# kekley/octree_pathtracing

Measured on AMD Instinct MI355X. Metric: Mrays/sec at 1920×1080×256spp; achieved HBM GB/s vs roofline at 1/2/4/8 GPUs, higher is better.
Workload: dtype f32

## Files before the change

octree_pathtracing_amd/csrc/octpt_api.cpp:

```cpp
#include <hip/hip_runtime.h>

#include <algorithm>
#include <atomic>
#include <chrono>
#include <cmath>
#include <cstdlib>
#include <thread>
#include <cstdio>
#include <cstring>
#include <new>
#include <string>
#include <memory>
#include <vector>

#include "../../include/octpt.h"
#include "octpt_internal.h"
#include "octpt_mask.h"
#include "octpt_reproject.h"

using namespace octpt;

namespace {

constexpr uint32_t kCounterRing = 256;
constexpr uint64_t kMaxChunkPaths = 1ull << 31;
constexpr uint64_t kDefaultChunkPaths = 1ull << 29;
#ifndef OCTPT_LOOKAHEAD
#define OCTPT_LOOKAHEAD 3
#endif
constexpr uint32_t kLookahead = OCTPT_LOOKAHEAD;
constexpr uint32_t kDefaultPool = 512u << 20;
constexpr uint32_t kMaxPool = 1u << 30;
constexpr uint32_t kMinPool = 1u << 20;
constexpr uint32_t kDefaultRefill = 0;
constexpr uint32_t kDefaultDrainRays = 4096;
#ifndef OCTPT_SAMPLE_GROUP_DEFAULT
#define OCTPT_SAMPLE_GROUP_DEFAULT 4
#endif
constexpr uint32_t kDefaultSampleGroup = OCTPT_SAMPLE_GROUP_DEFAULT;
constexpr uint64_t kGroupMinItems = 1ull << 27;

uint32_t group_shift_of(uint32_t most, uint32_t chunk_spp) {
    uint32_t g = 6u;
    while (g && ((1u << g) > most || chunk_spp % (1u << g) != 0u)) g -= 2u;
    return g;
}

uint32_t env_u32(const char *name, uint32_t dflt) {
    const char *v = std::getenv(name);
    if (!v || !*v) return dflt;
    const long x = std::strtol(v, nullptr, 10);
    return x > 0 ? (uint32_t)x : dflt;
}

struct EventPair {
    hipEvent_t start, stop;
};

template <class T>
struct DevBuf {
    T *p = nullptr;
    size_t n = 0;
};

}

struct octpt_ctx {
    int device = 0;
    int num_cu = 0;
    hipStream_t stream = nullptr;
    std::string err;
    bool has_scene = false;
    DevScene S{};
    std::vector<void *> scene_allocs;
    bool has_camera = false;
    octpt_camera cam{};
    DevCamera C{};
    uint32_t *d_counters = nullptr;
    std::vector<uint2> h_subs;
    uint2 *d_subs = nullptr;
    size_t subs_cap = 0;
    float *d_beam = nullptr;
    size_t beam_cap = 0;
    uint32_t launch_seq = 0;
    unsigned long long *d_stats = nullptr;
    uint8_t *d_lut_byte = nullptr;
    float *d_lut_float = nullptr;
    std::vector<EventPair> pending;
    double kernel_ms = 0.0;
    uint64_t launches = 0;
    bool ktiming = false;
    std::vector<std::pair<int, EventPair>> kpending;
    std::vector<EventPair> ev_pool;
    double kern_ms[2] = {0.0, 0.0};
    uint64_t kern_n[2] = {0, 0};
    float build_ms = 0.0f;
    BuildScratch build_scratch;
    int blocks_per_cu_cache[kMaxDepth + 1] = {0};
    int extend_bpc_cache[kMaxDepth + 1][4] = {};
    int shade_bpc_cache[2][2][3] = {};
    bool lean_scene = false;
    bool no_lean = false;
    bool sample_group_set = false;
    uint32_t sample_group = kDefaultSampleGroup;
    WaveBuffers wb{};
    size_t pool = 0, color_cap = 0, nee_pool = 0;
    void *nee_alloc = nullptr;
    std::vector<void *> wave_allocs;
    void *color_alloc = nullptr;
    size_t wave_bytes = 0, mem_limit = 0;
    std::vector<std::pair<void *, size_t>> wave_sizes;
    uint64_t wave_allocs_n = 0;
    bool oom_warned = false;
    uint32_t *h_count = nullptr;
    uint32_t *d_count = nullptr;
    hipEvent_t count_ev[kLookahead + 1] = {};
    uint32_t pool_cap = kDefaultPool, refill = kDefaultRefill;
    bool beam = true;
    uint32_t drain_rays = kDefaultDrainRays;
    bool drain_models = false;
    uint64_t chunk_cap = kDefaultChunkPaths;
    octpt_frame *inflight = nullptr;
    std::vector<octpt_ctx *> sub;
    float4 *m_acc = nullptr;
    uint32_t *m_seg = nullptr;
    size_t m_acc_cap = 0, m_seg_cap = 0;
    float4 *dn_frame[2] = {nullptr, nullptr};
    size_t dn_cap[2] = {0, 0};
    std::vector<uint32_t> h_order;
    uint32_t order_w = 0, order_h = 0;
    uint32_t *d_order = nullptr, *d_order_pos = nullptr;
    uint64_t scene_gen = 0, camera_gen = 0, order_gen = 0;
    struct BeamKey {
        uint64_t scene = 0, camera = 0, order = 0;
        uint64_t list = 0;
        uint32_t w = 0, h = 0, shard_index = 0, shard_count = 0;
        bool valid = false;
        bool operator==(const BeamKey &o) const {
            return valid && o.valid && scene == o.scene && camera == o.camera && order == o.order && list == o.list &&
                   w == o.w && h == o.h && shard_index == o.shard_index && shard_count == o.shard_count;
        }
    } beam_key;
    uint32_t *d_tiles = nullptr;
    size_t tiles_cap = 0;
    uint64_t list_gen = 0;
    uint32_t *d_tile_spp = nullptr;
    float *d_tile_err = nullptr;
    size_t tile_spp_cap = 0, tile_err_cap = 0;
    float sample_clamp = 0.0f;
    float *d_tile_spread = nullptr;
    size_t tile_spread_cap = 0;
    float4 *fin_normal = nullptr, *fin_albedo = nullptr;
    float *fin_depth = nullptr, *fin_var = nullptr;
    size_t fin_normal_cap = 0, fin_albedo_cap = 0, fin_depth_cap = 0, fin_var_cap = 0;
    hipEvent_t beam_ev = nullptr;
    hipStream_t beam_stream = nullptr;
    bool beam_shared = false;
};

struct octpt_frame {
    octpt_ctx *ctx = nullptr;
    octpt_render_params params{};
    std::thread worker;
    std::atomic<bool> finished{false};
    std::atomic<bool> cancel_requested{false};
    octpt_status status = OCTPT_OK;
    float *user_accum = nullptr;
    uint8_t *user_rgba = nullptr;
    size_t n_pixels = 0;
    float4 *d_accum = nullptr;
    uchar4 *d_rgba = nullptr;
    float *h_accum = nullptr;
    uint8_t *h_rgba = nullptr;
    bool delivered = false;
};

namespace {

octpt_status fail(octpt_ctx *ctx, octpt_status st, const std::string &msg) {
    if (ctx) ctx->err = msg;
    return st;
}

octpt_status hip_fail(octpt_ctx *ctx, hipError_t e, const char *what) {
    return fail(ctx, e == hipErrorOutOfMemory ? OCTPT_ERR_OOM : OCTPT_ERR_DEVICE,
                std::string(what) + ": " + hipGetErrorString(e));
}

#define HIP_TRY(ctx, expr)                                 \
    do {                                                   \
// ... 3155 lines not shown
```

octree_pathtracing_amd/csrc/octpt_kernels.hip:

```cpp
#include "octpt_internal.h"
#include "octpt_rcp.h"
#include "octpt_reproject.h"

#ifndef OCTPT_RCP_FAST
#define OCTPT_RCP_FAST 1
#endif

namespace octpt {
namespace {

#define RAY_EPSILON 0.00000005f
#define RAY_OFFSET 0.000001f
#define OCTREE_MAX_STEPS 1000u
#define OCTREE_MAX_SCALE 23u
#define OCTREE_EPSILON 1.1920929e-7f
#define MAX_DST_WORLD 1024.0f
#define PI_F 3.14159265358979323846f
#define CELL_TOL 0.001f
#define SUN_MAX_CHANCE 0.9f
#define MAT_FLAG_REFRACTIVE 0x4u
#define MAT_FLAG_SUBSURFACE 0x2u
#define MAX_PATH_SEGMENTS 64u
constexpr uint32_t kBeamIterBits = 10u;
constexpr uint32_t kBeamIterMask = (1u << kBeamIterBits) - 1u;
static_assert(OCTREE_MAX_STEPS <= kBeamIterMask + 1u, "the skipped-iteration bound fits its bits");

struct v3 {
    float x, y, z;
};
__device__ __forceinline__ v3 V(float x, float y, float z) { return v3{x, y, z}; }
__device__ __forceinline__ v3 vadd(v3 a, v3 b) { return V(a.x + b.x, a.y + b.y, a.z + b.z); }
__device__ __forceinline__ v3 vsub(v3 a, v3 b) { return V(a.x - b.x, a.y - b.y, a.z - b.z); }
__device__ __forceinline__ v3 vmul(v3 a, v3 b) { return V(a.x * b.x, a.y * b.y, a.z * b.z); }
__device__ __forceinline__ v3 vscale(v3 a, float s) { return V(a.x * s, a.y * s, a.z * s); }
__device__ __forceinline__ float vdot(v3 a, v3 b) { return (a.x * b.x + a.y * b.y) + a.z * b.z; }
__device__ __forceinline__ v3 vcross(v3 a, v3 b) {
    return V(a.y * b.z - b.y * a.z, a.z * b.x - b.z * a.x, a.x * b.y - b.x * a.y);
}
__device__ __forceinline__ v3 vnorm(v3 a) {
    float r = 1.0f / sqrtf(vdot(a, a));
    return vscale(a, r);
}
__device__ __forceinline__ float fmn(float a, float b) { return a < b ? a : b; }
__device__ __forceinline__ float fmx(float a, float b) { return a > b ? a : b; }
__device__ __forceinline__ float vmin3(v3 a) { return fmn(fmn(a.x, a.y), a.z); }
__device__ __forceinline__ float vmax3(v3 a) { return fmx(fmx(a.x, a.y), a.z); }
__device__ __forceinline__ float tmn(float a, float b) { return __builtin_fminf(a, b); }
__device__ __forceinline__ float tmx(float a, float b) { return __builtin_fmaxf(a, b); }
__device__ __forceinline__ float tmin3(v3 a) { return tmn(tmn(a.x, a.y), a.z); }
__device__ __forceinline__ float tmn_nc(float a, float b) {
    float r;
    asm("v_min_f32 %0, %1, %2" : "=v"(r) : "v"(a), "v"(b));
    return r;
}
__device__ __forceinline__ float tmax3(v3 a) { return tmx(tmx(a.x, a.y), a.z); }
__device__ __forceinline__ float signum_(float f) { return (__float_as_uint(f) >> 31) ? -1.0f : 1.0f; }

__device__ __forceinline__ void dm_sincos(float x, float &s, float &c) {
    const float kf = floorf(x * 0.636619772367581343f + 0.5f);
    const int k = (int)kf;
    const float r = ((x - kf * 1.5703125f) - kf * 4.837512969970703125e-4f) - kf * 7.54978995489188216e-8f;
    const float z = r * r;
    const float sp = r + r * z * (-1.6666654611e-1f + z * (8.3321608736e-3f + z * -1.9515295891e-4f));
    const float cp = (1.0f - 0.5f * z) +
                     z * z * (4.166664568298827e-2f + z * (-1.388731625493765e-3f + z * 2.443315711809948e-5f));
    switch (k & 3) {
    case 0: s = sp; c = cp; break;
    case 1: s = cp; c = -sp; break;
    case 2: s = -sp; c = -cp; break;
    default: s = -cp; c = sp; break;
    }
}
__device__ __forceinline__ float dm_cos(float x) { float s, c; dm_sincos(x, s, c); return c; }

__device__ inline float dm_asin(float x) {
    const float a = fabsf(x);
    float z, xx;
    bool flag = false;
    if (a > 0.5f) {
        z = 0.5f * (1.0f - a);
        xx = sqrtf(z);
        flag = true;
    } else {
        xx = a;
        z = a * a;
    }
    float r;
    if (a < 1.0e-4f && !flag) {
        r = xx;
    } else {
        r = ((((4.2163199048e-2f * z + 2.4181311049e-2f) * z + 4.5470025998e-2f) * z + 7.4953002686e-2f) * z +
             1.6666752422e-1f) * z * xx + xx;
    }
    if (flag) {
        r = r + r;
        r = 1.5707963267948966f - r;
    }
    return x < 0.0f ? -r : r;
}
__device__ inline float dm_acos(float x) {
    if (x < -0.5f) return PI_F - 2.0f * dm_asin(sqrtf(0.5f * (1.0f + x)));
    if (x > 0.5f) return 2.0f * dm_asin(sqrtf(0.5f * (1.0f - x)));
    return 1.5707963267948966f - dm_asin(x);
}
__device__ inline float dm_atan_core(float x) {
    float sgn = 1.0f, y;
    if (x < 0.0f) { sgn = -1.0f; x = -x; }
    if (x > 2.414213562373095f) {
        y = 1.5707963267948966f;
        x = -1.0f / x;
    } else if (x > 0.4142135623730950f) {
        y = 0.7853981633974483f;
        x = (x - 1.0f) / (x + 1.0f);
    } else {
        y = 0.0f;
    }
    const float z = x * x;
    y = y + ((((8.05374449538e-2f * z - 1.38776856032e-1f) * z + 1.99777106478e-1f) * z - 3.33329491539e-1f) * z * x + x);
    return sgn < 0.0f ? -y : y;
}
__device__ inline float dm_atan2(float y, float x) {
    int code = 0;
    if (x < 0.0f) code = 2;
    if (y < 0.0f) code |= 1;
    if (x == 0.0f) {
        if (code & 1) return -1.5707963267948966f;
        if (y == 0.0f) return 0.0f;
        return 1.5707963267948966f;
    }
    if (y == 0.0f) return (code & 2) ? PI_F : 0.0f;
    float w = 0.0f;
    if (code == 2) w = PI_F;
    else if (code == 3) w = -PI_F;
    return w + dm_atan_core(y / x);
}
__device__ __forceinline__ float dm_hypot(float x, float y) { return sqrtf(x * x + y * y); }

__device__ __forceinline__ uint32_t lowbias32(uint32_t x) {
    x ^= x >> 16; x *= 0x7feb352du; x ^= x >> 15; x *= 0x846ca68bu; x ^= x >> 16;
    return x;
}
__device__ __forceinline__ uint32_t path_state(uint32_t seed, uint32_t pixel, uint32_t sample) {
    uint32_t h = lowbias32(seed ^ 0xA511E9B3u);
    h = lowbias32(h ^ pixel);
    return lowbias32(h ^ (sample * 0x9E3779B9u));
}
__device__ __forceinline__ float rng_next(uint32_t &st) {
    const uint32_t s = st * 747796405u + 2891336453u;
    st = s;
    uint32_t w = ((s >> ((s >> 28u) + 4u)) ^ s) * 277803737u;
    w = (w >> 22u) ^ w;
    return (float)(w >> 8) * (1.0f / 16777216.0f);
}

__device__ __forceinline__ uint32_t branch_state(uint32_t state, uint32_t b) {
// ... 1355 lines not shown
    Counters cnt = {0u, 0u, 0u, 0u, 0u, 0u, 0u};
    const uint32_t item = blockIdx.x * kBlock + threadIdx.x;
    uint32_t x = 0u, y = 0u;
    if (item < R.total_items) item_pixel(R, item, x, y);
    if (item < R.total_items && x < R.W && y < R.H) {
        const uint32_t pix = y * R.W + x;
        PathState ps;
        const float xn = ((float)(2u * x + 1u) - (float)R.W) / R.dim;
        const float yn = ((float)(2u * (R.H - y) - 1u) - (float)R.H) / R.dim;
        const v3 nd = vadd(vadd(vscale(V(C.dir[0], C.dir[1], C.dir[2]), C.d_factor),
                                vscale(V(C.right[0], C.right[1], C.right[2]), xn)),
                           vscale(V(C.up[0], C.up[1], C.up[2]), yn));
        ps.o = V(C.eye[0], C.eye[1], C.eye[2]);
        ps.d = vnorm(nd);
        ps.n = V(0.0f, 0.0f, 0.0f);
        ps.col[0] = ps.col[1] = ps.col[2] = ps.col[3] = 0.0f;
        ps.T = V(1.0f, 1.0f, 1.0f);
        ps.L = V(0.0f, 0.0f, 0.0f);
        ps.cur = ps.prev = ps.depth = 0u;
        ps.rng = 0u;
        ps.last_prim = kPrimNone;
        ps.path_segs = 0u;
        ps.specular = true;
        cnt.paths++;
        uint32_t pix_segs = 0u;
        while (begin_segment(ps)) {
            cnt.segs++;
            pix_segs++;
            const TraceRay tr = trace_ray_of(S, ps);
            Esvo E;
            esvo_begin(S, tr, E, stk);
            uint32_t prim = kPrimNone;
            PrimHit h;
            int rs;
            do {
                rs = esvo_step<kPrims>(S, tr, E, stk, cnt, prim, h);
            } while (rs == kStepContinue);
            cnt.steps += E.iter;
            if (rs != kStepHit) break;
            commit_hit(S, ps, prim, h, cnt);
            if (ps.cur != 0u && ps.col[3] > 0.0f) break;
            ps.o = vadd(ps.o, vscale(ps.d, RAY_OFFSET));
        }
        float out[3];
        if (ps.cur == 0u) {
            sky_color(S.sun, ps, out);
        } else {
            const float shading = fmaxf(0.3f, vdot(ps.n, V(S.sun.sw[0], S.sun.sw[1], S.sun.sw[2])));
            for (int i = 0; i < 3; ++i) out[i] = ps.col[i] * (S.sun.emit[i] * shading);
        }
        const uint32_t ai = R.compact ? item : pix;
        float4 fb = accum[ai];
        fb.x = out[0];
        fb.y = out[1];
        fb.z = out[2];
        accum[ai] = fb;
        if (segcount) segcount[ai] += pix_segs;
    }
    cnt.ib = 0u;
    flush_counters(cnt, stats);
}

constexpr uint32_t kRayBeamBit = 0x40000000u;
constexpr uint32_t kHitCapped = 1u;
__device__ __forceinline__ void store_ray(const WaveBuffers &B, uint32_t q, uint32_t pos, uint32_t slot,
                                          const PathState &ps) {
    const bool beam = ps.beam > 0.0f && ps.path_segs == 1u;
    B.ray0[q][pos] = make_float4(ps.o.x, ps.o.y, ps.o.z, beam ? ps.beam : __uint_as_float(ps.last_prim));
    B.ray1[q][pos] = make_float4(ps.d.x, ps.d.y, ps.d.z,
                                 __uint_as_float(slot | (vdot(ps.d, ps.n) < 0.0f ? 0x80000000u : 0u) |
                                                 (beam ? kRayBeamBit : 0u)));
}
__device__ __forceinline__ void store_cam_ray(const WaveBuffers &B, uint32_t pos, const PathState &ps) {
    B.ray1[0][pos] = make_float4(ps.d.x, ps.d.y, ps.d.z, ps.beam > 0.0f ? ps.beam : 0.0f);
}
__device__ __forceinline__ void cam_ray(float4 eye, uint32_t slot, float4 &r0, float4 &r1) {
    const float b = r1.w;
    r0 = make_float4(eye.x, eye.y, eye.z, b > 0.0f ? b : eye.w);
    r1.w = __uint_as_float(slot | (b > 0.0f ? kRayBeamBit : 0u));
}
__device__ __forceinline__ uint32_t ray_last_prim(float4 r0, float4 r1) {
    return (__float_as_uint(r1.w) & kRayBeamBit) ? kPrimNone : __float_as_uint(r0.w);
}
__device__ __forceinline__ float ray_beam(float4 r0, float4 r1) {
    return (__float_as_uint(r1.w) & kRayBeamBit) ? r0.w : 0.0f;
}

__device__ __forceinline__ void pack_path(const PathState &ps, uint32_t item, float4 &a, float4 &b, uint2 &c) {
    a = make_float4(ps.T.x, ps.T.y, ps.T.z, ps.L.x);
    b = make_float4(ps.L.y, ps.L.z, __uint_as_float(ps.rng), __uint_as_float(item));
    c = make_uint2(ps.cur, ps.depth | (ps.specular ? 1u << 8 : 0u) | (ps.shadow ? 1u << 9 : 0u) | (ps.branch << 10) |
                               (ps.path_segs << 16) | (ps.seg_base << 23));
}
__device__ __forceinline__ void store_path(const WaveBuffers &B, uint32_t slot, const PathState &ps, uint32_t item) {
    float4 a, b;
    uint2 c;
    pack_path(ps, item, a, b, c);
    B.pa[slot] = a;
    B.pb[slot] = b;
    B.pc[slot] = c;
}

__device__ __forceinline__ void store_lean_at(const WaveBuffers &B, uint32_t q, uint32_t pos, const PathState &ps) {
    float4 a, b;
    uint2 c;
    pack_path(ps, 0u, a, b, c);
    (q ? B.pb : B.pa)[pos] = make_float4(a.x, a.y, a.z, b.z);
    B.pc[(size_t)q * kSegs * B.seg_cap + pos] = c;
}

__device__ __forceinline__ void store_nee(const WaveBuffers &B, uint32_t slot, const PathState &ps) {
    B.pd[slot] = make_float4(ps.co.x, ps.co.y, ps.co.z, __uint_as_float(ps.clast));
    B.pd[B.pool + slot] = make_float4(ps.cd.x, ps.cd.y, ps.cd.z, __uint_as_float(ps.ccur));
    B.pd[2u * B.pool + slot] = make_float4(ps.cn.x, ps.cn.y, ps.cn.z, ps.mult);
}
__device__ __forceinline__ void store_att(const WaveBuffers &B, uint32_t slot, const PathState &ps) {
    B.pd[3u * B.pool + slot] = make_float4(ps.att[0], ps.att[1], ps.att[2], ps.att[3]);
}
__device__ __forceinline__ void load_nee(const WaveBuffers &B, uint32_t slot, PathState &ps) {
    const float4 a = B.pd[slot], b = B.pd[B.pool + slot], c = B.pd[2u * B.pool + slot], d = B.pd[3u * B.pool + slot];
    ps.co = V(a.x, a.y, a.z);
    ps.clast = __float_as_uint(a.w);
    ps.cd = V(b.x, b.y, b.z);
    ps.ccur = __float_as_uint(b.w);
    ps.cn = V(c.x, c.y, c.z);
    ps.mult = c.w;
    ps.att[0] = d.x; ps.att[1] = d.y; ps.att[2] = d.z; ps.att[3] = d.w;
}

__device__ __forceinline__ void unpack_path(float4 a, float4 b, uint2 c, float4 r0, float4 r1, PathState &ps,
                                            uint32_t &item) {
    ps.o = V(r0.x, r0.y, r0.z);
    ps.last_prim = ray_last_prim(r0, r1);
    ps.d = V(r1.x, r1.y, r1.z);
    ps.beam = 0.0f;
    ps.T = V(a.x, a.y, a.z);
    ps.L = V(a.w, b.x, b.y);
    ps.rng = __float_as_uint(b.z);
    item = __float_as_uint(b.w);
    ps.cur = c.x;
    ps.prev = c.x;
    ps.depth = c.y & 255u;
    ps.specular = (c.y >> 8) & 1u;
    ps.shadow = (c.y >> 9) & 1u;
    ps.branch = (c.y >> 10) & 63u;
    ps.path_segs = (c.y >> 16) & 127u;
    ps.seg_base = c.y >> 23;
}
__device__ __forceinline__ void load_path(const WaveBuffers &B, uint32_t slot, float4 r0, float4 r1, PathState &ps,
                                          uint32_t &item) {
    unpack_path(B.pa[slot], B.pb[slot], B.pc[slot], r0, r1, ps, item);
}

__device__ __forceinline__ uint32_t group_swap(uint32_t v, uint32_t pos, uint32_t low) {
    const uint32_t mid = (v >> pos) & 7u;
    return (v & ~(7u << pos)) | ((((mid & ((1u << low) - 1u)) << (3u - low)) | (mid >> low)) << pos);
}
template <bool kFastDiv = true>
__device__ __forceinline__ void item_split(const DevRender &R, uint32_t item, uint32_t &s_local, uint32_t &px_item) {
    const uint32_t g = R.group_shift;
    const uint32_t n = item >> g;
    const uint32_t sg = kFastDiv ? udiv_c(n, R.div_items) : n / R.total_items;
    const uint32_t pq = n - sg * R.total_items;
    s_local = (sg << g) | (item & ((1u << g) - 1u));
    px_item = g ? group_swap(pq, 3u - (g >> 1), 3u - (g >> 1)) : pq;
}
__device__ __forceinline__ size_t item_of(const DevRender &R, uint32_t s_local, uint32_t pq) {
    const uint32_t g = R.group_shift;
    return (((size_t)(s_local >> g) * R.total_items + pq) << g) + (s_local & ((1u << g) - 1u));
}

template <bool kFastDiv = true>
__device__ __forceinline__ bool item_path(const DevCamera &C, const DevRender &R, uint32_t item, PathState &ps,
                                          uint32_t &x, uint32_t &y) {
    uint32_t s_local, px_item;
    item_split<kFastDiv>(R, item, s_local, px_item);
    item_pixel<kFastDiv>(R, px_item, x, y);
    if (x >= R.W || y >= R.H) return false;
    uint32_t sample = R.spp_start + s_local, branch = 0u;
    if (R.subs) {
        const uint2 sb = R.subs[s_local];
        sample = sb.x;
        branch = sb.y >> 16;
    }
    new_path(C, R, x, y, sample, ps);
    ps.branch = branch;
    begin_segment(ps);
    return true;
}

template <bool kSeed = false>
__device__ inline bool seed_item(const DevCamera &C, const DevRender &R, const WaveBuffers &B, uint32_t slot,
                                 uint32_t item, PathState &ps, Counters &cnt) {
    uint32_t x, y;
    if (!item_path(C, R, item, ps, x, y)) {
        B.color[item] = make_float4(0.0f, 0.0f, 0.0f, 0.0f);
        return false;
    }
    cnt.paths++;
    if (R.beam)
        ps.beam = R.beam[(y / kBeamTile) * R.beam_tx + x / kBeamTile];
    if (kSeed) {
        if (!B.lean) B.item0[slot] = item;
    } else {
        store_path(B, slot, ps, item);
    }
    return true;
}

static_assert(kSegs == 64, "segment scans give one wave lane per segment");

__device__ __forceinline__ uint32_t relaxed_load(const uint32_t *p) {
    return __hip_atomic_load(p, __ATOMIC_RELAXED, __HIP_MEMORY_SCOPE_AGENT);
}
__device__ __forceinline__ uint32_t shard_lo(uint32_t k, uint32_t n) {
    return (uint32_t)(((uint64_t)k * n) / kSegs);
}
__device__ __forceinline__ uint32_t first_from(uint64_t m, uint32_t from) {
    const uint64_t r = from ? ((m >> from) | (m << (64u - from))) : m;
    return (from + (uint32_t)__ffsll((unsigned long long)r) - 1u) & 63u;
}

struct ItemCursor {
    uint32_t k;
    bool left;
};

template <bool kSeed = false>
__device__ inline bool regen(const DevCamera &C, const DevRender &R, const WaveBuffers &B, uint32_t slot, bool want,
                             uint32_t chunk_items, ItemCursor &cur, PathState &ps, Counters &cnt) {
    bool need = want, ok = false;
    while (cur.left && __ballot(need) != 0ull) {
        const uint32_t lo = shard_lo(cur.k, chunk_items), n = shard_lo(cur.k + 1u, chunk_items) - lo;
        const uint32_t t = wave_ticket(B.ctrl + ctr_item(cur.k), need);
        bool dry = false;
        if (need) {
            if (t >= n) dry = true;
            else if (seed_item<kSeed>(C, R, B, slot, lo + t, ps, cnt)) { ok = true; need = false; }
        }
        if (__ballot(dry) != 0ull) {
            const uint32_t j = threadIdx.x & 63u;
            const bool has = relaxed_load(B.ctrl + ctr_item(j)) < shard_lo(j + 1u, chunk_items) - shard_lo(j, chunk_items);
            const uint64_t m = __ballot(has);
            cur.left = m != 0ull;
            if (cur.left) cur.k = first_from(m, cur.k);
        }
    }
    return ok;
}

__global__ __launch_bounds__(kBlock) void wf_seed_kernel(DevCamera C, DevRender R, WaveBuffers B, uint32_t n_seed,
                                                         uint32_t chunk_items, unsigned long long *__restrict__ stats) {
    const uint32_t i = blockIdx.x * kBlock + threadIdx.x;
    const uint32_t seg = (i >> 6) % kSegs;
    Counters cnt = {0u, 0u, 0u, 0u, 0u, 0u, 0u};
    PathState ps;
    bool ok = false;
    uint32_t slot = i;
    if (n_seed == chunk_items) {
        if (blockIdx.x == 0u && threadIdx.x < kSegs)
            B.ctrl[ctr_item(threadIdx.x)] = shard_lo(threadIdx.x + 1u, chunk_items) - shard_lo(threadIdx.x, chunk_items);
        const uint32_t lo = shard_lo(seg, chunk_items), hi = shard_lo(seg + 1u, chunk_items);
        const uint32_t item = lo + (i >> 6) / kSegs * 64u + (i & 63u);
        slot = item;
        if (item < hi) ok = seed_item<true>(C, R, B, slot, item, ps, cnt);
        if (((R.W | R.H) & (kTile - 1u)) == 0u) {
            if (blockIdx.x == 0u && threadIdx.x < kSegs)
                B.ctrl[ctr_count(0u, threadIdx.x)] = shard_lo(threadIdx.x + 1u, chunk_items) - shard_lo(threadIdx.x, chunk_items);
            if (ok) store_cam_ray(B, seg * B.seg_cap + (item - lo), ps);
            if (blockIdx.x == 0u && threadIdx.x == 0u) B.ray0[0][0] = B.eye;
            if (blockIdx.x == 0u && threadIdx.x == 0u) atomicAdd(&stats[kStatPaths], (unsigned long long)chunk_items);
            return;
        }
    } else {
        ItemCursor cur = {seg, true};
        ok = regen<true>(C, R, B, i, i < n_seed, chunk_items, cur, ps, cnt);
    }
    const uint32_t t = wave_ticket(B.ctrl + ctr_count(0u, seg), ok);
    if (ok) store_ray(B, 0u, seg * B.seg_cap + t, slot, ps);
    flush_counters(cnt, stats);
}

#ifndef OCTPT_SPH_WAVES
#define OCTPT_SPH_WAVES 8
#endif
#ifndef OCTPT_BOX_WAVES
#define OCTPT_BOX_WAVES 7
#endif
#ifndef OCTPT_MDL_WAVES
#define OCTPT_MDL_WAVES 6
#endif
#ifndef OCTPT_BLK_WAVES
#define OCTPT_BLK_WAVES 6
#endif
#define OCTPT_EXTEND_WAVES_OF(k)                                                                              \
    ((k) == kPrimsSpheres ? OCTPT_SPH_WAVES                                                                   \
                          : (k) == kPrimsBoxes ? OCTPT_BOX_WAVES : (k) == kPrimsBlocks ? OCTPT_BLK_WAVES : OCTPT_MDL_WAVES)
#ifndef OCTPT_CLAIM
#define OCTPT_CLAIM 64
#endif
constexpr uint32_t kClaim = OCTPT_CLAIM;
static_assert(kSegs % 8u == 0u, "eight XCDs share the segments evenly");
#ifndef OCTPT_THR_LONG
#define OCTPT_THR_LONG 16
#endif
#ifndef OCTPT_THR_SHORT
#define OCTPT_THR_SHORT 32
#endif
#ifndef OCTPT_SHORT_STEPS
#define OCTPT_SHORT_STEPS 48
// ... 237 lines not shown
        if (valid) {
            float4 r1 = B.ray1[q][i];
            if (first == 2u) {
                float4 r0c;
                cam_ray(B.eye, shard_lo(seg, chunk_items) + base + lane, r0c, r1);
            }
            const float4 r0 = first ? B.eye : B.ray0[q][i];
            append = shade_lane<kNee, kMode == 2, kSP>(S, C, R, B, first != 0u, r0, r1, B.hit + i,
                                                  S.has_blocks ? B.hit4 + i : nullptr, ps, slot, item, cnt, q, i);
            finished = !append;
        }
        if constexpr (kMode == 1) {
            if (regen(C, R, B, slot, finished, chunk_items, cur, ps, cnt)) append = true;
        }
        const uint32_t t = wave_ticket(B.ctrl + ctr_count(q ^ 1u, seg), append);
        if (append) {
            store_ray(B, q ^ 1u, seg0 + t, slot, ps);
            if constexpr (kMode == 2) store_lean_at(B, q ^ 1u, seg0 + t, ps);
        }
    }
    cnt.ib = 0u;
    flush_counters(cnt, stats);
}

template <int kPrims, bool kNee>
__global__ __launch_bounds__(kBlock) void wf_drain_kernel(DevScene S, DevRender R, WaveBuffers B, uint32_t q,
                                                          unsigned long long *__restrict__ stats) {
    extern __shared__ uint2 lds_stack[];
    const Stack stk = stack_of(lds_stack, S.depth);
    Counters cnt = {0u, 0u, 0u, 0u, 0u, 0u, 0u};
    const uint32_t wid = (blockIdx.x * kBlock + threadIdx.x) >> 6, nw = (gridDim.x * kBlock) >> 6;
    const uint32_t jlim = (threadIdx.x & 63u) == 0u ? 0xFFFFFFFFu : 0u;
    for (uint32_t k = 0; k < kSegs; ++k) {
        const uint32_t n = min(B.ctrl[ctr_count(q, k)], jlim);
        for (uint32_t j = wid; j < n; j += nw) {
            const uint32_t p = k * B.seg_cap + j;
            float4 r0 = B.ray0[q][p], r1 = B.ray1[q][p];
            for (;;) {
                const TraceRay tr = make_trace_ray(S, V(r0.x, r0.y, r0.z), V(r1.x, r1.y, r1.z), ray_last_prim(r0, r1),
                                                   (__float_as_uint(r1.w) >> 31) != 0u);
                Esvo E;
                esvo_begin(S, tr, E, stk, ray_beam(r0, r1));
                cnt.steps -= E.iter;
                bool beam_ray = (__float_as_uint(r1.w) & kRayBeamBit) != 0u;
                uint32_t prim = kPrimNone;
                PrimHit h;
                int rs;
                for (;;) {
                    do {
                        HIT_POISON(prim, h);
                        rs = esvo_step<kPrims, true>(S, tr, E, stk, cnt, prim, h);
                        SLOT_CHECK(E, stats, kStatDrainRow);
                    } while (rs == kStepContinue);
                    HIT_CHECK(kPrims, rs, prim, h, stats, kStatDrainRow);
                    cnt.steps += E.iter;
                    if (!((rs == kStepMiss) & esvo_capped(E.iter) & beam_ray)) break;
                    cnt.redo++;
                    beam_ray = false;
                    esvo_root(S, E);
                    esvo_first_child(E);
                }
                cnt.segs++;
                uint2 hr;
                if constexpr (kPrims == kPrimsBlocks)
                    hr = rs == kStepHit ? make_uint2(prim, __float_as_uint(h.t)) : make_uint2(kPrimNone, 0u);
                else
                    hr = rs == kStepHit ? hit_record(prim, h) : make_uint2(kPrimNone, 0u);
                const uint4 h4 = make_uint4(hr.x, hr.y, __float_as_uint(h.u), __float_as_uint(h.v));
                PathState ps;
                uint32_t slot, item;
                const bool lean = !kNee && B.lean;
                const bool cont = lean ? shade_lane<kNee, true>(S, DevCamera{}, R, B, false, r0, r1, &hr, &h4, ps, slot, item,
                                                                cnt, q, p)
                                       : shade_lane<kNee, false>(S, DevCamera{}, R, B, false, r0, r1, &hr, &h4, ps, slot, item, cnt);
                if (!cont) break;
                if (lean) store_lean_at(B, q, p, ps);
                r0 = make_float4(ps.o.x, ps.o.y, ps.o.z, __uint_as_float(ps.last_prim));
                r1 = make_float4(ps.d.x, ps.d.y, ps.d.z,
                                 __uint_as_float(slot | (vdot(ps.d, ps.n) < 0.0f ? 0x80000000u : 0u)));
            }
        }
    }
    flush_counters(cnt, stats, kStatDrainRow);
}

__device__ __forceinline__ float luminance(float r, float g, float b);

__device__ __forceinline__ void running_moments(float2 &m, v3 c, uint32_t spp, uint32_t bc) {
    const float s_inv = 1.0f / (float)(bc + spp);
    const float fs = (float)spp, w = (float)bc;
    const float l = luminance(c.x, c.y, c.z);
    m.x = (m.x * fs + l * w) * s_inv;
    m.y = (m.y * fs + (l * l) * w) * s_inv;
}

__device__ __forceinline__ v3 clamp_sample(v3 c, float clamp) {
    const float l = luminance(c.x, c.y, c.z);
    if (l > clamp) {
        const float k = clamp / l;
        c = V(c.x * k, c.y * k, c.z * k);
    }
    return c;
}

template <bool kMoments, bool kClamp>
__device__ __forceinline__ void resolve_pixel(const DevRender &R, const WaveBuffers &B, uint32_t chunk_spp,
                                              float4 *__restrict__ accum, uint32_t *__restrict__ segcount,
                                              float2 *__restrict__ moments, float clamp) {
    const uint32_t px_item = blockIdx.x * kBlock + threadIdx.x;
    if (px_item >= R.total_items) return;
    uint32_t x, y;
    item_pixel(R, px_item, x, y);
    if (x >= R.W || y >= R.H) return;
    const uint32_t acc_idx = R.compact ? px_item : y * R.W + x;
    float4 fb = accum[acc_idx];
    float2 mo = make_float2(0.0f, 0.0f);
    if constexpr (kMoments) mo = moments[acc_idx];
    uint32_t segs = 0u;
    v3 L0 = V(0.0f, 0.0f, 0.0f), sum = L0;
    bool split = false;
    const uint32_t gh = R.group_shift >> 1;
    const uint32_t pq = gh ? group_swap(px_item, 3u - gh, gh) : px_item;
    for (uint32_t s = 0; s < chunk_spp; ++s) {
        const float4 c = B.color[item_of(R, s, pq)];
        const uint32_t w = __float_as_uint(c.w);
        segs += w & 0x7FFFFFFFu;
        if (!R.subs) {
            v3 cs = V(c.x, c.y, c.z);
            if constexpr (kClamp) cs = clamp_sample(cs, clamp);
            running_mean(fb, cs, R.spp_start + s, 1u);
            if constexpr (kMoments) running_moments(mo, cs, R.spp_start + s, 1u);
            continue;
        }
        const uint2 sb = R.subs[s];
        const uint32_t b = sb.y >> 16, bc = sb.y & 0xFFFFu;
        if (b == 0u) {
            L0 = V(c.x, c.y, c.z);
            sum = vadd(V(0.0f, 0.0f, 0.0f), L0);
            split = (w >> 31) != 0u;
        } else {
            sum = vadd(sum, V(c.x, c.y, c.z));
        }
        if (b + 1u == bc) {
            const float inv = 1.0f / (float)bc;
            v3 folded = split ? vscale(sum, inv) : L0;
            if constexpr (kClamp) folded = clamp_sample(folded, clamp);
            running_mean(fb, folded, sb.x, bc);
            if constexpr (kMoments) running_moments(mo, folded, sb.x, bc);
        }
    }
    accum[acc_idx] = fb;
    if constexpr (kMoments) moments[acc_idx] = mo;
    if (segcount) segcount[acc_idx] += segs;
}

__global__ __launch_bounds__(kBlock) void wf_resolve_kernel(DevRender R, WaveBuffers B, uint32_t chunk_spp,
                                                            float4 *__restrict__ accum, uint32_t *__restrict__ segcount) {
    resolve_pixel<false, false>(R, B, chunk_spp, accum, segcount, nullptr, 0.0f);
}

__global__ __launch_bounds__(kBlock) void wf_resolve_moments_kernel(DevRender R, WaveBuffers B, uint32_t chunk_spp,
                                                                    float4 *__restrict__ accum,
                                                                    uint32_t *__restrict__ segcount,
                                                                    float2 *__restrict__ moments) {
    resolve_pixel<true, false>(R, B, chunk_spp, accum, segcount, moments, 0.0f);
}

__global__ __launch_bounds__(kBlock) void wf_resolve_clamp_kernel(DevRender R, WaveBuffers B, uint32_t chunk_spp,
                                                                  float4 *__restrict__ accum,
                                                                  uint32_t *__restrict__ segcount, float clamp) {
    resolve_pixel<false, true>(R, B, chunk_spp, accum, segcount, nullptr, clamp);
}

__global__ __launch_bounds__(kBlock) void wf_resolve_moments_clamp_kernel(DevRender R, WaveBuffers B, uint32_t chunk_spp,
                                                                          float4 *__restrict__ accum,
                                                                          uint32_t *__restrict__ segcount,
                                                                          float2 *__restrict__ moments, float clamp) {
    resolve_pixel<true, true>(R, B, chunk_spp, accum, segcount, moments, clamp);
}

template <int kPrims>
__global__ __launch_bounds__(kBlock) void intersect_kernel(DevScene S, const float *__restrict__ rays,
                                                           const uint32_t *__restrict__ last_prim,
                                                           const float *__restrict__ last_normal, uint32_t n,
                                                           float *__restrict__ out_t, uint32_t *__restrict__ out_prim,
                                                           float *__restrict__ out_normal, uint32_t *__restrict__ out_steps) {
    extern __shared__ uint2 lds_stack[];
    const Stack stk = stack_of(lds_stack, S.depth);
    const uint32_t i = blockIdx.x * kBlock + threadIdx.x;
    if (i >= n) return;
    PathState ps;
    ps.o = V(rays[6 * i], rays[6 * i + 1], rays[6 * i + 2]);
    ps.d = V(rays[6 * i + 3], rays[6 * i + 4], rays[6 * i + 5]);
    ps.n = last_normal ? V(last_normal[3 * i], last_normal[3 * i + 1], last_normal[3 * i + 2]) : V(0.0f, 0.0f, 0.0f);
    ps.cur = ps.prev = ps.depth = 0u;
    ps.last_prim = last_prim ? last_prim[i] : kPrimNone;
    ps.specular = true;
    const TraceRay tr = trace_ray_of(S, ps);
    Esvo E;
    Counters cnt = {0u, 0u, 0u, 0u, 0u, 0u, 0u};
    esvo_begin(S, tr, E, stk);
    uint32_t prim = kPrimNone;
    PrimHit h;
    int rs;
    do {
        rs = esvo_step<kPrims>(S, tr, E, stk, cnt, prim, h);
    } while (rs == kStepContinue);
    if (rs == kStepHit) {
        commit_hit(S, ps, prim, h, cnt);
        out_t[i] = h.t;
        out_prim[i] = kPrims != kPrimsBlocks ? prim : ((prim & kPrimCuboidBit) ? kQuadKey | (prim & kPrimIndexMask)
                                                                                 : prim & kPrimIndexMask);
        if (out_normal) {
            out_normal[3 * i] = ps.n.x;
            out_normal[3 * i + 1] = ps.n.y;
            out_normal[3 * i + 2] = ps.n.z;
        }
    } else {
        out_t[i] = __int_as_float(0x7f800000);
        out_prim[i] = kPrimNone;
        if (out_normal) out_normal[3 * i] = out_normal[3 * i + 1] = out_normal[3 * i + 2] = 0.0f;
    }
    if (out_steps) out_steps[i] = E.iter;
}

constexpr int kBeamLevels = 24;
static_assert(kTile % kBeamTile == 0, "beam tiles nest in the 8x8 render tiles");
constexpr uint32_t kBeamSub = (kTile / kBeamTile) * (kTile / kBeamTile);
__host__ __device__ constexpr uint32_t beam_levels(uint32_t depth) {
    return depth < 1u ? 1u : depth < (uint32_t)kBeamLevels ? depth : (uint32_t)kBeamLevels;
}
#ifndef OCTPT_BEAM_VISITS
#define OCTPT_BEAM_VISITS (1u << 13)
#endif
constexpr uint32_t kBeamVisits = OCTPT_BEAM_VISITS;
#ifndef OCTPT_BEAM_LOD
#define OCTPT_BEAM_LOD 0.0f
#endif
constexpr float kBeamLod = OCTPT_BEAM_LOD;
constexpr float kBeamEsvoSlack = 0x1p-21f;

__device__ __forceinline__ float beam_pack(float t, uint32_t nodes) {
    const uint32_t bound = 4u * nodes;
    const uint32_t b = __float_as_uint(t);
    if (bound >= OCTREE_MAX_STEPS || b < 2u * (kBeamIterMask + 1u)) return 0.0f;
    return __uint_as_float(((b - (kBeamIterMask + 1u)) & ~kBeamIterMask) | bound);
}

constexpr uint32_t kBeamLanes = 8u;
__global__ __launch_bounds__(64) void beam_kernel(DevScene S, DevCamera C, DevRender R, uint32_t n_tiles,
                                                  float *__restrict__ beam) {
    const uint32_t lane = threadIdx.x & (kBeamLanes - 1u), grp = threadIdx.x / kBeamLanes;
    const uint32_t i = blockIdx.x * (64u / kBeamLanes) + grp;
    if (i >= n_tiles) return;
    const uint32_t rt = dealt_tile(R.tile_order, R.shard_index + (i / kBeamSub) * R.shard_count), sub = i % kBeamSub;
    const uint32_t rty = udiv_c(rt, R.div_tiles_x);
    const uint32_t x0 = (rt - rty * R.tiles_x) * kTile + (sub % (kTile / kBeamTile)) * kBeamTile,
                   y0 = rty * kTile + (sub / (kTile / kBeamTile)) * kBeamTile;
    if (x0 >= R.W || y0 >= R.H) return;
    const uint32_t tile = (y0 / kBeamTile) * R.beam_tx + x0 / kBeamTile;
    const uint32_t x1 = min(x0 + kBeamTile, R.W), y1 = min(y0 + kBeamTile, R.H);
    float s0 = ((float)(2u * x0) - (float)R.W) / R.dim, s1 = ((float)(2u * x1) - (float)R.W) / R.dim;
    float t0 = ((float)(2u * (R.H - y1)) - (float)R.H) / R.dim, t1 = ((float)(2u * (R.H - y0)) - (float)R.H) / R.dim;
    const float ps = 0.02f * (s1 - s0) + 1e-6f, pt = 0.02f * (t1 - t0) + 1e-6f;
    s0 -= ps; s1 += ps; t0 -= pt; t1 += pt;
    const v3 F = vscale(V(C.dir[0], C.dir[1], C.dir[2]), C.d_factor);
    const v3 Rt = V(C.right[0], C.right[1], C.right[2]), Up = V(C.up[0], C.up[1], C.up[2]);
    const v3 Ek[4] = {vadd(vadd(F, vscale(Rt, s0)), vscale(Up, t0)), vadd(vadd(F, vscale(Rt, s1)), vscale(Up, t0)),
                      vadd(vadd(F, vscale(Rt, s1)), vscale(Up, t1)), vadd(vadd(F, vscale(Rt, s0)), vscale(Up, t1))};
    const v3 Ec = vadd(vadd(F, vscale(Rt, 0.5f * (s0 + s1))), vscale(Up, 0.5f * (t0 + t1)));
    v3 pn[4];
    for (int k = 0; k < 4; ++k) {
        v3 n = vcross(Ek[k], Ek[(k + 1) & 3]);
        if (vdot(n, Ec) < 0.0f) n = vscale(n, -1.0f);
        pn[k] = n;
    }
    const v3 e = vadd(vscale(V(C.eye[0], C.eye[1], C.eye[2]), S.octree_scale), V(1.0f, 1.0f, 1.0f));
    const float slack = kBeamEsvoSlack * (4.0f + fmaxf(fmaxf(fabsf(e.x), fabsf(e.y)), fabsf(e.z)));
    auto box = [&](v3 lo, float h) -> float {
        const v3 a = vsub(lo, e), b = vsub(vadd(lo, V(h, h, h)), e);
        const float ext = fmaxf(fmaxf(fmaxf(fabsf(a.x), fabsf(b.x)), fmaxf(fabsf(a.y), fabsf(b.y))),
                                fmaxf(fabsf(a.z), fabsf(b.z)));
        for (int k = 0; k < 4; ++k) {
            const v3 n = pn[k];
            const float mx = (fmaxf(n.x * a.x, n.x * b.x) + fmaxf(n.y * a.y, n.y * b.y)) + fmaxf(n.z * a.z, n.z * b.z);
            const float tol = (1e-5f * ext + slack) * ((fabsf(n.x) + fabsf(n.y)) + fabsf(n.z));
            if (mx < -tol) return -1.0f;
        }
        const float dx = a.x > 0.0f ? a.x : (b.x < 0.0f ? -b.x : 0.0f);
        const float dy = a.y > 0.0f ? a.y : (b.y < 0.0f ? -b.y : 0.0f);
        const float dz = a.z > 0.0f ? a.z : (b.z < 0.0f ? -b.z : 0.0f);
        return sqrtf((dx * dx + dy * dy) + dz * dz);
    };
    const float lod = kBeamLod * fmaxf(s1 - s0, t1 - t0) / sqrtf(vdot(F, F));
    float best = __builtin_inff();
    extern __shared__ uint32_t beam_lds[];
    const uint32_t t = threadIdx.x, L = beam_levels(S.depth);
    constexpr uint32_t G = 64u / kBeamLanes;
    float *const st_d = reinterpret_cast<float *>(beam_lds);
    uint32_t *const st_base = beam_lds + L * 64u, *const st_mask = st_base + L * G;
    float *const st_lx = reinterpret_cast<float *>(st_mask + L * G), *const st_ly = st_lx + L * G, *const st_lz = st_ly + L * G;
    auto grp_min = [](uint32_t k) {
        k = min(k, (uint32_t)__builtin_amdgcn_update_dpp((int)k, (int)k, 0xB1, 0xF, 0xF, false));
        k = min(k, (uint32_t)__builtin_amdgcn_update_dpp((int)k, (int)k, 0x4E, 0xF, 0xF, false));
        k = min(k, (uint32_t)__builtin_amdgcn_update_dpp((int)k, (int)k, 0x141, 0xF, 0xF, false));
        return k;
// ... 625 lines not shown

hipError_t launch_denoise_prep(uint32_t W, uint32_t H, const float4 *color, const float4 *albedo, const float *depth,
                               float4 *sig, hipStream_t stream) {
    const uint32_t n = W * H;
    hipLaunchKernelGGL(denoise_prep_kernel, dim3((n + 255u) / 256u), dim3(256), 0, stream, n, color, albedo, depth, sig);
    return hipGetLastError();
}

hipError_t launch_atrous(const DevDenoise &D, uint32_t iter, bool last, const float4 *src, float4 *dst,
                         hipStream_t stream) {
    const dim3 grid((D.W + kDnX - 1u) / kDnX, (D.H + kDnY - 1u) / kDnY);
    hipLaunchKernelGGL(last ? atrous_kernel<true> : atrous_kernel<false>, grid, dim3(256), 0, stream, D, iter, src, dst);
    return hipGetLastError();
}

hipError_t launch_temporal(const DevTemporal &T, bool moments, hipStream_t stream) {
    const dim3 grid((T.W + kDnX - 1u) / kDnX, (T.H + kDnY - 1u) / kDnY);
    hipLaunchKernelGGL(moments ? temporal_kernel<true> : temporal_kernel<false>, grid, dim3(256), 0, stream, T);
    return hipGetLastError();
}

hipError_t launch_variance(const DevVariance &V, hipStream_t stream) {
    const dim3 grid((V.W + kDnX - 1u) / kDnX, (V.H + kDnY - 1u) / kDnY);
    hipLaunchKernelGGL(variance_kernel, grid, dim3(256), 0, stream, V);
    return hipGetLastError();
}

hipError_t launch_denoise_var_prep(uint32_t W, uint32_t H, const float4 *color, const float *variance,
                                   const float4 *albedo, const float *depth, float4 *sig, hipStream_t stream) {
    const uint32_t n = W * H;
    hipLaunchKernelGGL(denoise_var_prep_kernel, dim3((n + 255u) / 256u), dim3(256), 0, stream, n, color, variance, albedo,
                       depth, sig);
    return hipGetLastError();
}

hipError_t launch_atrous_var(const DevDenoiseVar &D, uint32_t iter, bool last, const float4 *src, float4 *dst,
                             hipStream_t stream) {
    const dim3 grid((D.W + kDnX - 1u) / kDnX, (D.H + kDnY - 1u) / kDnY);
    hipLaunchKernelGGL(last ? atrous_var_kernel<true> : atrous_var_kernel<false>, grid, dim3(256), 0, stream, D, iter, src,
                       dst);
    return hipGetLastError();
}

hipError_t launch_render(const DevScene &S0, const DevCamera &C, const DevRender &R, float4 *accum, uint32_t *segcount,
                         uint32_t *counter, unsigned long long *stats, int grid, hipStream_t stream) {
    const DevScene &S = S0;
    auto kern = S.sun.sun_sampling ? (S.has_blocks ? render_kernel<true, kPrimsBlocks> : render_kernel<true, kPrimsModels>)
                                   : (S.has_blocks ? render_kernel<false, kPrimsBlocks> : render_kernel<false, kPrimsModels>);
    hipLaunchKernelGGL(kern, dim3(grid), dim3(kBlock), render_lds_bytes(S.depth), stream, S, C, R, accum, segcount,
                       counter, stats);
    return hipGetLastError();
}

hipError_t launch_wf_seed(const DevCamera &C, const DevRender &R, const WaveBuffers &B, uint32_t n_seed,
                          uint32_t chunk_items, unsigned long long *stats, hipStream_t stream) {
    const uint64_t threads = n_seed == chunk_items
                                 ? (uint64_t)kSegs * ((((uint64_t)chunk_items + kSegs - 1u) / kSegs + 63u) / 64u) * 64u
                                 : (uint64_t)n_seed;
    hipLaunchKernelGGL(wf_seed_kernel, dim3((uint32_t)((threads + kBlock - 1u) / kBlock)), dim3(kBlock), 0, stream, C, R, B, n_seed,
                       chunk_items, stats);
    return hipGetLastError();
}

hipError_t launch_wf_extend(const DevScene &S, const WaveBuffers &B, uint32_t q, bool cam, uint32_t refill, int grid,
                            unsigned long long *stats, hipStream_t stream) {
    uint32_t rf = refill | (cam ? 0x80000000u : 0u);
    void *args[] = {const_cast<DevScene *>(&S), const_cast<WaveBuffers *>(&B), &q, &rf, &stats};
    const hipError_t e = hipLaunchKernel(extend_instance(S), dim3(grid), dim3(kBlock), args, render_lds_bytes(S.depth),
                                         stream);
    if (e != hipSuccess) return e;
    return hipGetLastError();
}

template <bool kLds, int kSP>
static const void *lean_shade_of(bool first) {
    return !first ? reinterpret_cast<const void *>(wf_shade_kernel<false, kLds, 2, true, kSP>)
                  : reinterpret_cast<const void *>(wf_shade_kernel<false, kLds, 2, false, kSP>);
}
template <bool kNee, bool kLds>
static const void *shade_instance_of(int mode, bool first, int prims) {
    if (!kNee && mode == 2) {
        if (prims == kShadeSphColour) return lean_shade_of<kLds, kShadeSphColour>(first);
        if (prims == kPrimsSpheres) return lean_shade_of<kLds, kPrimsSpheres>(first);
        if (prims == kPrimsBoxes) return lean_shade_of<kLds, kPrimsBoxes>(first);
        if (prims == kPrimsBlocks) return lean_shade_of<kLds, kPrimsBlocks>(first);
        return lean_shade_of<kLds, kPrimsModels>(first);
    }
    return mode == 1 ? reinterpret_cast<const void *>(wf_shade_kernel<kNee, kLds, 1>)
                     : reinterpret_cast<const void *>(wf_shade_kernel<kNee, kLds, 0>);
}
bool shade_lds_tables(const DevScene &S) { return S.n_mats <= kShadeLdsMats && S.n_texs <= kShadeLdsMats; }
static const void *shade_instance(const DevScene &S, int mode, bool first = false) {
    const bool lds = shade_lds_tables(S);
    const int prims = S.has_blocks    ? kPrimsBlocks
                      : S.has_models  ? kPrimsModels
                      : S.has_cuboids ? kPrimsBoxes
                      : S.has_images  ? kPrimsSpheres
                                      : kShadeSphColour;
    return S.sun.sun_sampling
               ? (lds ? shade_instance_of<true, true>(mode, first, prims) : shade_instance_of<true, false>(mode, first, prims))
               : (lds ? shade_instance_of<false, true>(mode, first, prims) : shade_instance_of<false, false>(mode, first, prims));
}

int shade_blocks_per_cu(const DevScene &S, int mode) {
    int blocks = 0;
    if (hipOccupancyMaxActiveBlocksPerMultiprocessor(&blocks, shade_instance(S, mode), kBlock, 0) != hipSuccess)
        return 4;
    return blocks > 0 ? blocks : 1;
}

hipError_t launch_wf_shade(const DevScene &S, const DevCamera &C, const DevRender &R, const WaveBuffers &B, uint32_t q,
                           uint32_t chunk_items, uint32_t first, bool regen, int grid, unsigned long long *stats,
                           hipStream_t stream) {
    uint32_t first_u = first;
    void *args[] = {const_cast<DevScene *>(&S), const_cast<DevCamera *>(&C), const_cast<DevRender *>(&R),
                    const_cast<WaveBuffers *>(&B), &q, &chunk_items, &first_u, &stats};
    const hipError_t e = hipLaunchKernel(shade_instance(S, shade_mode(regen, B.lean != 0u), first != 0u), dim3(grid),
                                         dim3(kBlock), args, 0, stream);
    if (e != hipSuccess) return e;
    return hipGetLastError();
}

hipError_t launch_wf_drain(const DevScene &S, const DevRender &R, const WaveBuffers &B, uint32_t q, int grid,
                           unsigned long long *stats, hipStream_t stream) {
    const bool nee = S.sun.sun_sampling != 0;
    const void *fn = S.has_blocks ? (nee ? reinterpret_cast<const void *>(wf_drain_kernel<kPrimsBlocks, true>)
                                         : reinterpret_cast<const void *>(wf_drain_kernel<kPrimsBlocks, false>))
                     : S.has_models ? (nee ? reinterpret_cast<const void *>(wf_drain_kernel<kPrimsModels, true>)
                                         : reinterpret_cast<const void *>(wf_drain_kernel<kPrimsModels, false>))
                     : S.has_cuboids ? (nee ? reinterpret_cast<const void *>(wf_drain_kernel<kPrimsBoxes, true>)
                                            : reinterpret_cast<const void *>(wf_drain_kernel<kPrimsBoxes, false>))
                                     : (nee ? reinterpret_cast<const void *>(wf_drain_kernel<kPrimsSpheres, true>)
                                            : reinterpret_cast<const void *>(wf_drain_kernel<kPrimsSpheres, false>));
    void *args[] = {const_cast<DevScene *>(&S), const_cast<DevRender *>(&R), const_cast<WaveBuffers *>(&B), &q, &stats};
    const hipError_t e = hipLaunchKernel(fn, dim3(grid), dim3(kBlock), args, render_lds_bytes(S.depth), stream);
    if (e != hipSuccess) return e;
    return hipGetLastError();
}

__global__ __launch_bounds__(2 * kSegs) void wf_snapshot_kernel(const uint32_t *__restrict__ ctrl, uint32_t q,
                                                                uint32_t *__restrict__ host_out) {
    const uint32_t t = threadIdx.x;
    host_out[t] = ctrl[t < kSegs ? ctr_count(q, t) : ctr_item(t - kSegs)];
}

hipError_t launch_wf_snapshot(const WaveBuffers &B, uint32_t q, uint32_t *host_out, hipStream_t stream) {
    hipLaunchKernelGGL(wf_snapshot_kernel, dim3(1), dim3(2 * kSegs), 0, stream, B.ctrl, q, host_out);
    return hipGetLastError();
}

hipError_t launch_wf_resolve(const DevRender &R, const WaveBuffers &B, uint32_t chunk_spp, float4 *accum,
                             uint32_t *segcount, float2 *moments, float clamp, hipStream_t stream) {
    const dim3 grid((R.total_items + kBlock - 1u) / kBlock);
    if (clamp != 0.0f) {
        if (moments)
            hipLaunchKernelGGL(wf_resolve_moments_clamp_kernel, grid, dim3(kBlock), 0, stream, R, B, chunk_spp, accum,
                               segcount, moments, clamp);
        else
            hipLaunchKernelGGL(wf_resolve_clamp_kernel, grid, dim3(kBlock), 0, stream, R, B, chunk_spp, accum, segcount,
                               clamp);
    } else if (moments)
        hipLaunchKernelGGL(wf_resolve_moments_kernel, grid, dim3(kBlock), 0, stream, R, B, chunk_spp, accum, segcount,
                           moments);
    else
        hipLaunchKernelGGL(wf_resolve_kernel, grid, dim3(kBlock), 0, stream, R, B, chunk_spp, accum, segcount);
    return hipGetLastError();
}

hipError_t launch_adaptive_init(uint32_t n, float4 *accum, float2 *moments, hipStream_t stream) {
    hipLaunchKernelGGL(adaptive_init_kernel, dim3((n + 255u) / 256u), dim3(256), 0, stream, n, accum, moments);
    return hipGetLastError();
}

hipError_t launch_tile_error(uint32_t W, uint32_t H, float luminance_floor, const float2 *moments,
                             const uint32_t *tile_spp, float *error, hipStream_t stream) {
    const uint32_t tiles_x = (W + kTile - 1u) / kTile, n_tiles = tiles_x * ((H + kTile - 1u) / kTile);
    const uint32_t per_block = kBlock / 64u;
    hipLaunchKernelGGL(tile_error_kernel, dim3((n_tiles + per_block - 1u) / per_block), dim3(kBlock), 0, stream, W, H,
                       tiles_x, n_tiles, luminance_floor, moments, tile_spp, error);
    return hipGetLastError();
}

hipError_t launch_tile_error_spread(uint32_t W, uint32_t H, float w, const float *error, float *out, hipStream_t stream) {
    const uint32_t tiles_x = (W + kTile - 1u) / kTile, tiles_y = (H + kTile - 1u) / kTile;
    hipLaunchKernelGGL(tile_error_spread_kernel, dim3((tiles_x * tiles_y + 255u) / 256u), dim3(256), 0, stream, tiles_x,
                       tiles_y, w, error, out);
    return hipGetLastError();
}

hipError_t launch_sample_variance(uint32_t W, uint32_t H, const float2 *moments, const uint32_t *tile_spp,
                                  const float *depth, const float4 *albedo, float *out, hipStream_t stream) {
    hipLaunchKernelGGL(sample_variance_kernel, dim3((W * H + 255u) / 256u), dim3(256), 0, stream, W, H,
                       (W + kTile - 1u) / kTile, moments, tile_spp, depth, albedo, out);
    return hipGetLastError();
}

hipError_t launch_intersect(const DevScene &S0, const float *rays, const uint32_t *last_prim, const float *last_normal,
                            uint32_t n, float *t, uint32_t *prim, float *normal, uint32_t *steps, hipStream_t stream) {
    const DevScene &S = S0;
    const uint32_t grid = (n + kBlock - 1u) / kBlock;
    hipLaunchKernelGGL(S.has_blocks ? intersect_kernel<kPrimsBlocks> : intersect_kernel<kPrimsModels>, dim3(grid),
                       dim3(kBlock), render_lds_bytes(S.depth), stream, S, rays, last_prim, last_normal, n, t, prim,
                       normal, steps);
    return hipGetLastError();
}

hipError_t launch_beam(const DevScene &S, const DevCamera &C, const DevRender &R, float *beam, hipStream_t stream) {
    const uint32_t n = R.shard_tiles * kBeamSub;
    const size_t lds = (64u + 5u * (64u / kBeamLanes)) * beam_levels(S.depth) * sizeof(uint32_t);
    const uint32_t per_block = 64u / kBeamLanes;
    hipLaunchKernelGGL(beam_kernel, dim3((n + per_block - 1u) / per_block), dim3(64), lds, stream, S, C, R, n, beam);
    return hipGetLastError();
}

hipError_t launch_tonemap(const float4 *accum, uchar4 *out, uint32_t n, const uint8_t *lut_byte, hipStream_t stream) {
    hipLaunchKernelGGL(tonemap_kernel, dim3((n + 255u) / 256u), dim3(256), 0, stream, accum, out, n, lut_byte);
    return hipGetLastError();
}

hipError_t launch_multi_stage(const DevRender &R, uint32_t n_dev, uint32_t stride, float4 *accum, uint32_t *seg,
                              float4 *stage_accum, uint32_t *stage_seg, bool to_stage, hipStream_t stream) {
    hipLaunchKernelGGL(multi_stage_kernel, dim3((R.total_items + 255u) / 256u), dim3(256), 0, stream, R, n_dev, stride,
                       accum, seg, stage_accum, stage_seg, to_stage ? 1u : 0u);
    return hipGetLastError();
}

hipError_t launch_unshard(uint32_t W, uint32_t H, uint32_t shard_count, const uint32_t *tile_pos, const float4 *shards,
                          uint32_t stride, float4 *frame, hipStream_t stream) {
    hipLaunchKernelGGL(unshard_kernel, dim3((W * H + 255u) / 256u), dim3(256), 0, stream, W, H, shard_count, tile_pos,
                       shards, stride, frame);
    return hipGetLastError();
}

}
```

Before: 5305.

## Add LDS-transposed wide resolve kernel and raise default sample group to 64

Adds a resolve kernel for grouped sample layouts. Each wave loads contiguous color records in coalesced batches, transposes them through padded LDS, then folds the samples per pixel. This targets the strided, poorly coalesced global reads the per-pixel resolve did when samples are interleaved in groups. The default sample group rises from 4 to 64, which changes the item ordering for the whole wavefront pipeline and may hurt trace coherence or exceed group limits for some spp settings.

```diff
diff --git a/octree_pathtracing_amd/csrc/octpt_api.cpp b/octree_pathtracing_amd/csrc/octpt_api.cpp
--- a/octree_pathtracing_amd/csrc/octpt_api.cpp
+++ b/octree_pathtracing_amd/csrc/octpt_api.cpp
@@ -35,7 +35,7 @@
 constexpr uint32_t kDefaultRefill = 0;
 constexpr uint32_t kDefaultDrainRays = 4096;
 #ifndef OCTPT_SAMPLE_GROUP_DEFAULT
-#define OCTPT_SAMPLE_GROUP_DEFAULT 4
+#define OCTPT_SAMPLE_GROUP_DEFAULT 64
 #endif
 constexpr uint32_t kDefaultSampleGroup = OCTPT_SAMPLE_GROUP_DEFAULT;
 constexpr uint64_t kGroupMinItems = 1ull << 27;
diff --git a/octree_pathtracing_amd/csrc/octpt_kernels.hip b/octree_pathtracing_amd/csrc/octpt_kernels.hip
--- a/octree_pathtracing_amd/csrc/octpt_kernels.hip
+++ b/octree_pathtracing_amd/csrc/octpt_kernels.hip
@@ -1,6 +1,7 @@
 #include "octpt_internal.h"
 #include "octpt_rcp.h"
 #include "octpt_reproject.h"
+#include "octpt_resolve_map.h"
 
 #ifndef OCTPT_RCP_FAST
 #define OCTPT_RCP_FAST 1
@@ -1662,10 +1663,6 @@
     unpack_path(B.pa[slot], B.pb[slot], B.pc[slot], r0, r1, ps, item);
 }
 
-__device__ __forceinline__ uint32_t group_swap(uint32_t v, uint32_t pos, uint32_t low) {
-    const uint32_t mid = (v >> pos) & 7u;
-    return (v & ~(7u << pos)) | ((((mid & ((1u << low) - 1u)) << (3u - low)) | (mid >> low)) << pos);
-}
 template <bool kFastDiv = true>
 __device__ __forceinline__ void item_split(const DevRender &R, uint32_t item, uint32_t &s_local, uint32_t &px_item) {
     const uint32_t g = R.group_shift;
@@ -2209,6 +2206,80 @@
     accum[acc_idx] = fb;
     if constexpr (kMoments) moments[acc_idx] = mo;
     if (segcount) segcount[acc_idx] += segs;
+}
+
+template <bool kMoments, bool kClamp, uint32_t K>
+__device__ __forceinline__ void resolve_pixel_wide(const DevRender &R, const WaveBuffers &B, uint32_t chunk_spp,
+                                                   float4 *__restrict__ accum, uint32_t *__restrict__ segcount,
+                                                   float2 *__restrict__ moments, float clamp, float4 *stage) {
+    const uint32_t px_item = blockIdx.x * kBlock + threadIdx.x;
+    if (px_item >= R.total_items) return;
+    const uint32_t lane = threadIdx.x & 63u;
+    float4 *st = stage + (threadIdx.x >> 6) * resolve_wave_slots(K);
+    uint32_t x, y;
+    item_pixel(R, px_item, x, y);
+    const bool live = x < R.W && y < R.H;
+    const uint32_t acc_idx = R.compact ? px_item : y * R.W + x;
+    float4 fb = make_float4(0.0f, 0.0f, 0.0f, 0.0f);
+    float2 mo = make_float2(0.0f, 0.0f);
+    if (live) {
+        fb = accum[acc_idx];
+        if constexpr (kMoments) mo = moments[acc_idx];
+    }
+    uint32_t segs = 0u;
+    const uint32_t g = R.group_shift, gh = g >> 1;
+    const uint32_t q = group_swap(px_item, 3u - gh, gh) & 63u;
+    uint32_t src[K], dst[K];
+#pragma unroll
+    for (uint32_t i = 0; i < K; ++i) {
+        src[i] = resolve_load_record(i, lane, K, g);
+        dst[i] = resolve_load_slot(i, lane, K);
+    }
+    const uint32_t n_groups = chunk_spp >> g;
+    for (uint32_t sg = 0; sg < n_groups; ++sg) {
+        const float4 *span = B.color + (((size_t)sg * R.total_items + (px_item & ~63u)) << g);
+        for (uint32_t j0 = 0; j0 < (1u << g); j0 += K) {
+            float4 c[K];
+#pragma unroll
+            for (uint32_t i = 0; i < K; ++i) c[i] = span[src[i] + j0];
+#pragma unroll
+            for (uint32_t i = 0; i < K; ++i) st[dst[i]] = c[i];
+            __builtin_amdgcn_fence(__ATOMIC_RELEASE, "workgroup");
+            __builtin_amdgcn_wave_barrier();
+            __builtin_amdgcn_fence(__ATOMIC_ACQUIRE, "workgroup");
+#pragma unroll
+            for (uint32_t k = 0; k < K; ++k) c[k] = st[resolve_read_slot(q, k, K)];
+            __builtin_amdgcn_fence(__ATOMIC_RELEASE, "workgroup");
+            __builtin_amdgcn_wave_barrier();
+            __builtin_amdgcn_fence(__ATOMIC_ACQUIRE, "workgroup");
+            if (!live) continue;
+#pragma unroll
+            for (uint32_t k = 0; k < K; ++k) {
+                const uint32_t s = (sg << g) + j0 + k;
+                segs += __float_as_uint(c[k].w) & 0x7FFFFFFFu;
+                v3 cs = V(c[k].x, c[k].y, c[k].z);
+                if constexpr (kClamp) cs = clamp_sample(cs, clamp);
+                running_mean(fb, cs, R.spp_start + s, 1u);
+                if constexpr (kMoments) running_moments(mo, cs, R.spp_start + s, 1u);
+            }
+        }
+    }
+    if (!live) return;
+    accum[acc_idx] = fb;
+    if constexpr (kMoments) moments[acc_idx] = mo;
+    if (segcount) segcount[acc_idx] += segs;
+}
+
+template <bool kMoments, bool kClamp>
+__global__ __launch_bounds__(kBlock) void wf_resolve_wide_kernel(DevRender R, WaveBuffers B, uint32_t chunk_spp,
+                                                                 float4 *__restrict__ accum,
+                                                                 uint32_t *__restrict__ segcount,
+                                                                 float2 *__restrict__ moments, float clamp) {
+    __shared__ float4 stage[(kBlock / 64u) * resolve_wave_slots(kResolveBatch)];
+    if (R.group_shift == 2u)
+        resolve_pixel_wide<kMoments, kClamp, 4u>(R, B, chunk_spp, accum, segcount, moments, clamp, stage);
+    else
+        resolve_pixel_wide<kMoments, kClamp, kResolveBatch>(R, B, chunk_spp, accum, segcount, moments, clamp, stage);
 }
 
 __global__ __launch_bounds__(kBlock) void wf_resolve_kernel(DevRender R, WaveBuffers B, uint32_t chunk_spp,
@@ -3140,6 +3211,22 @@
 hipError_t launch_wf_resolve(const DevRender &R, const WaveBuffers &B, uint32_t chunk_spp, float4 *accum,
                              uint32_t *segcount, float2 *moments, float clamp, hipStream_t stream) {
     const dim3 grid((R.total_items + kBlock - 1u) / kBlock);
+    if (R.group_shift != 0u) {
+        if (clamp != 0.0f) {
+            if (moments)
+                hipLaunchKernelGGL((wf_resolve_wide_kernel<true, true>), grid, dim3(kBlock), 0, stream, R, B, chunk_spp,
+                                   accum, segcount, moments, clamp);
+            else
+                hipLaunchKernelGGL((wf_resolve_wide_kernel<false, true>), grid, dim3(kBlock), 0, stream, R, B, chunk_spp,
+                                   accum, segcount, moments, clamp);
+        } else if (moments)
+            hipLaunchKernelGGL((wf_resolve_wide_kernel<true, false>), grid, dim3(kBlock), 0, stream, R, B, chunk_spp,
+                               accum, segcount, moments, clamp);
+        else
+            hipLaunchKernelGGL((wf_resolve_wide_kernel<false, false>), grid, dim3(kBlock), 0, stream, R, B, chunk_spp,
+                               accum, segcount, moments, clamp);
+        return hipGetLastError();
+    }
     if (clamp != 0.0f) {
         if (moments)
             hipLaunchKernelGGL(wf_resolve_moments_clamp_kernel, grid, dim3(kBlock), 0, stream, R, B, chunk_spp, accum,
diff --git a/octree_pathtracing_amd/csrc/octpt_resolve_map.h b/octree_pathtracing_amd/csrc/octpt_resolve_map.h
--- /dev/null
+++ b/octree_pathtracing_amd/csrc/octpt_resolve_map.h
@@ -0,0 +1,35 @@
+#pragma once
+#include <stdint.h>
+
+#if defined(__HIP__)
+#define OCTPT_MAP_FN __host__ __device__ inline __attribute__((always_inline))
+#else
+#define OCTPT_MAP_FN inline
+#endif
+
+namespace octpt {
+
+OCTPT_MAP_FN uint32_t group_swap(uint32_t v, uint32_t pos, uint32_t low) {
+    const uint32_t mid = (v >> pos) & 7u;
+    return (v & ~(7u << pos)) | ((((mid & ((1u << low) - 1u)) << (3u - low)) | (mid >> low)) << pos);
+}
+
+#ifndef OCTPT_RESOLVE_BATCH
+#define OCTPT_RESOLVE_BATCH 8
+#endif
+constexpr uint32_t kResolveBatch = OCTPT_RESOLVE_BATCH;
+static_assert(kResolveBatch == 4u || kResolveBatch == 8u || kResolveBatch == 16u, "a power of two, at most G = 16");
+
+OCTPT_MAP_FN constexpr uint32_t resolve_wave_slots(uint32_t K) { return 64u * (K + 1u); }
+
+OCTPT_MAP_FN uint32_t resolve_load_record(uint32_t i, uint32_t lane, uint32_t K, uint32_t g) {
+    const uint32_t r = i * 64u + lane;
+    return ((r / K) << g) + (r & (K - 1u));
+}
+OCTPT_MAP_FN uint32_t resolve_load_slot(uint32_t i, uint32_t lane, uint32_t K) {
+    const uint32_t r = i * 64u + lane;
+    return (r / K) * (K + 1u) + (r & (K - 1u));
+}
+OCTPT_MAP_FN uint32_t resolve_read_slot(uint32_t q, uint32_t k, uint32_t K) { return q * (K + 1u) + k; }
+
+}
```

New measurement: 5473 (median of 6 runs). 1.03x the previous value.
